# vliu15/speech-masters-thesis

Measured on AMD Instinct MI355X. Metric: LJSpeech utterances/sec per VQ-VAE train step, higher is better.
Workload: dtype bf16

## Files before the change

### include/smt_hip.h

```cpp
#ifndef SMT_HIP_H
#define SMT_HIP_H

#include <stddef.h>
#include <stdint.h>

#ifdef __cplusplus
extern "C" {
#endif

typedef void* smt_stream_t;

enum { SMT_F32 = 0, SMT_BF16 = 1 };

const char* smt_last_error(void);
int smt_abi_version(void);

size_t smt_vq_prep_bytes(int k_bins, int dim);
int smt_vq_prepare(const float* codebook, int k_bins, int dim, void* prep, size_t prep_bytes, smt_stream_t stream);

size_t smt_vq_forward_workspace_bytes(int64_t n_rows, int k_bins, int dim);
int smt_vq_forward(const float* x, const float* codebook, void* prep, const float* row_mask,
                   int64_t n_rows, int k_bins, int dim,
                   int64_t* idx, float* min_dist, float* x_d, float* sums,
                   void* workspace, size_t workspace_bytes, smt_stream_t stream);
// ... 56 lines not shown
  const int* lens_in2;
  int c_in2, ld_x2;
  int64_t bs_x2;
  const uint32_t* drop_keys_dev;
  int drop_keys_dev_stride;
} smt_conv_desc;
int smt_conv1d_ntc(const smt_conv_desc* desc, smt_stream_t stream);
const char* smt_conv1d_kernel_name(const smt_conv_desc* desc);

size_t smt_conv1d_wgrad_workspace_bytes(const smt_conv_desc* desc);
int smt_conv1d_wgrad(const smt_conv_desc* desc, float* dweight, int64_t stride_out, int64_t stride_in,
                     int64_t stride_tap, const int* tap_map, float* dbias, void* workspace,
                     size_t workspace_bytes, smt_stream_t stream);
int smt_wgrad_reduce_defer(int on, smt_stream_t stream);
const char* smt_conv1d_wgrad_kernel_name(const smt_conv_desc* desc);

size_t smt_conv1x1_bwd_workspace_bytes(const smt_conv_desc* desc);
int smt_conv1x1_bwd(const smt_conv_desc* desc, float* dweight, int64_t stride_out, int64_t stride_in, float* dbias,
                    void* workspace, size_t workspace_bytes, smt_stream_t stream);

size_t smt_conv_k1_bwd_workspace_bytes(int batch, int t);
int smt_conv_k1_bwd(const void* dh, int64_t bs_dh, int ld_dh, const void* x, int64_t bs_x, int ld_x,
                    const void* w_packed_bwd, const void* res, int64_t bs_res, int ld_res, void* dx, int64_t bs_dx,
                    int ld_dx, const int* lens, int batch, int t, const void* zero_page, float* dweight,
                    int64_t stride_out, int64_t stride_in, float* dbias, void* workspace, size_t workspace_bytes,
                    smt_stream_t stream);

int smt_convt4s2(const void* x, int64_t bs_x, int ld_x, const void* w_packed, const float* bias, void* y, int64_t bs_y,
                 int ld_y, const int* lens_in, const int* lens_out, int batch, int t_in, int c_out, const void* zero_page,
                 smt_stream_t stream);
int smt_conv4s2(const void* x, int64_t bs_x, int ld_x, const void* w_packed, const float* bias, void* y, int64_t bs_y,
                int ld_y, const int* lens_in, const int* lens_out, int batch, int t_in, int c_in, const void* zero_page,
                smt_stream_t stream);

// ... 137 lines not shown
```

### speech-masters-thesis_amd/csrc/common.hip

```cpp
#include <stdarg.h>

#include "smt_common.h"

namespace smt {
static thread_local char g_err[512] = "";
void set_error(const char* fmt, ...) {
  va_list ap;
  va_start(ap, fmt);
  vsnprintf(g_err, sizeof(g_err), fmt, ap);
  va_end(ap);
}
}

extern "C" const char* smt_last_error(void) { return smt::g_err; }
extern "C" int smt_abi_version(void) { return 5; }
```

### speech-masters-thesis_amd/csrc/conv1x1_bwd.hip

```cpp
#include <algorithm>

#include "conv_common.h"

namespace smt {

struct Bwd1x1Args {
  const void* dy; const void* u; const void* w; void* dx; float* slab;
  const int* lens_out;
  long long dy_bs, u_bs, dx_bs;
  int lddy, ldu, lddx;
  int B, T, tiles_per_batch, tiles_per_wg, with_bias;
  float scale;
};

constexpr int FB_ROWS = 128, FB_C = 128, FB_ROWB = FB_C * 2, FB_TILE = FB_ROWS * FB_ROWB, FB_NT = 512;
constexpr int FB_NDX = 2 * 2;

__device__ __forceinline__ int fb_swz(int row) { return ((row & 3) << 2) | ((row >> 2) & 3); }

__device__ __forceinline__ bf16x8 fb_tr2(const unsigned char* pa, const unsigned char* pb) {
  s16x4 lo = __builtin_amdgcn_ds_read_tr16_b64_v4i16((__attribute__((address_space(3))) s16x4*)pa);
  s16x4 hi = __builtin_amdgcn_ds_read_tr16_b64_v4i16((__attribute__((address_space(3))) s16x4*)pb);
  typedef short s16x8 __attribute__((ext_vector_type(8)));
  s16x8 v = {lo[0], lo[1], lo[2], lo[3], hi[0], hi[1], hi[2], hi[3]};
  return __builtin_bit_cast(bf16x8, v);
}

__global__ __launch_bounds__(FB_NT) void conv1x1_bwd_kernel(Bwd1x1Args p) {
  typedef __bf16 T;
  extern __shared__ __attribute__((aligned(1024))) unsigned char smem[];
  const int tid = threadIdx.x, lane = tid & 63, wave = tid >> 6;
  const int wm = wave >> 2, wn = wave & 3;
  const int r = lane & 31, hh = lane >> 5;

  const int ntiles = p.tiles_per_batch * p.B;
  const int nwg = gridDim.x;
  const int wg = (blockIdx.x & 7) * (nwg >> 3) + (blockIdx.x >> 3);
  const int tile_begin = min(ntiles, wg * p.tiles_per_wg);
  const int tile_end = min(ntiles, tile_begin + p.tiles_per_wg);

  bf16x8 wfrag[FB_C / 16];
  {
    const int ci = wn * 32 + r;
    const unsigned char* wrow = reinterpret_cast<const unsigned char*>(p.w) + (size_t)ci * FB_ROWB;
#pragma unroll
    for (int kk = 0; kk < FB_C / 16; ++kk)
      wfrag[kk] = *reinterpret_cast<const bf16x8*>(wrow + (((2 * kk + hh) ^ (ci & 15)) << 4));
  }

  float bsum[2] = {0.f, 0.f};
  f32x16 accw[2];
#pragma unroll
// ... 131 lines not shown
      out[(size_t)row * FB_C + wn * 32 + r] = accw[j][e];
    }
#pragma unroll
  for (int j = 0; j < 2; ++j) {
    const float other = __shfl_xor(bsum[j], 32);
    if (hh == 0) out[(size_t)(64 + 32 * j + r) * FB_C + 32 * wn] = bsum[j] + other;
  }
}

static int bwd1x1_nwg(const smt_conv_desc* d) {
  const long long ntiles = (long long)((d->t_out + FB_ROWS - 1) / FB_ROWS) * d->batch;
  long long nwg = std::min<long long>(256, std::max<long long>(8, (ntiles + fused_min_tpw() - 1) / fused_min_tpw()));
  return (int)((nwg + 7) / 8 * 8);
}

}

using namespace smt;

static bool bwd1x1_ok(const smt_conv_desc* d) {
  return d->dtype == SMT_BF16 && d->taps == 1 && d->c_in == FB_C && d->c_out == FB_C && d->stride == 1 &&
         d->dilation == 1 && d->padding == 0 && d->out_stride == 1 && d->out_offset == 0 && d->t_in == d->t_out &&
         d->t_y == d->t_out && d->w_swizzled && d->zero_page && d->act_grad && d->act_grad_src && !d->res &&
         !d->act_out && !d->bias && !d->lens_in;
}

extern "C" size_t smt_conv1x1_bwd_workspace_bytes(const smt_conv_desc* d) {
  if (!d) return 0;
  return (size_t)bwd1x1_nwg(d) * 2 * 2 * 64 * FB_C * sizeof(float);
}

extern "C" int smt_conv1x1_bwd(const smt_conv_desc* d, float* dweight, int64_t stride_out, int64_t stride_in,
                               float* dbias, void* workspace, size_t workspace_bytes, smt_stream_t stream_) {
  hipStream_t stream = (hipStream_t)stream_;
  SMT_CHECK_ARG(d && d->x && d->y && d->w && dweight && workspace, "smt_conv1x1_bwd: null pointer");
  SMT_CHECK_ARG(bwd1x1_ok(d),
                "smt_conv1x1_bwd: needs the bf16 1x1 data-gradient descriptor of a 128->128 layer (swizzled weights, "
                "zero_page, act_grad set, no bias/res/act_out/lens_in)");
  SMT_CHECK_ARG(d->ld_x % 8 == 0 && d->ld_y % 8 == 0 && d->ld_act % 8 == 0, "smt_conv1x1_bwd: row pitches must keep 16-byte alignment");
  SMT_CHECK_ARG(workspace_bytes >= smt_conv1x1_bwd_workspace_bytes(d), "smt_conv1x1_bwd: workspace too small");
  const int nwg = bwd1x1_nwg(d);
  if (d->batch > 0 && d->t_out > 0) {
    Bwd1x1Args a;
    a.dy = d->x; a.u = d->act_grad_src; a.w = d->w; a.dx = d->y; a.slab = (float*)workspace;
    a.lens_out = d->lens_out;
    a.dy_bs = d->bs_x; a.u_bs = d->bs_act; a.dx_bs = d->bs_y;
    a.lddy = d->ld_x; a.ldu = d->ld_act; a.lddx = d->ld_y;
    a.B = d->batch; a.T = d->t_out;
    a.tiles_per_batch = (d->t_out + FB_ROWS - 1) / FB_ROWS;
    const long long ntiles = (long long)a.tiles_per_batch * d->batch;
    a.tiles_per_wg = (int)((ntiles + nwg - 1) / nwg);
    a.with_bias = dbias ? 1 : 0;
    a.scale = d->drop_scale;
    (void)hipFuncSetAttribute((const void*)conv1x1_bwd_kernel, hipFuncAttributeMaxDynamicSharedMemorySize, 160 * 1024);
    conv1x1_bwd_kernel<<<nwg, FB_NT, 4 * FB_TILE, stream>>>(a);
    SMT_CHECK_LAUNCH("conv1x1_bwd");
  }
  const int jmap[1] = {0};
  const int n_chunks = (d->batch > 0 && d->t_out > 0) ? nwg : 0;
  return launch_wgrad_reduce((const float*)workspace, dweight, dbias, n_chunks, 2, 1, 1, FB_C, FB_C, FB_C, stride_out,
                             stride_in, 0, jmap, stream, 4);
}
```

### speech-masters-thesis_amd/csrc/conv_wgrad.hip

```cpp
#include <algorithm>
#include <cstdlib>

#include "conv_common.h"

namespace smt {

struct WgradArgs {
  const void* x; const void* dy; float* slab;
  const int* lens_in;
  long long x_bs, dy_bs;
  int ldx, ldy;
  int B, Tin, Tout, Ty, Cin, Cout;
  int taps, stride, dil, pad, out_stride, out_offset;
  int rows_per_chunk, chunks_per_batch, nblk_ci, nblk_co, with_bias;
  int rs;
  int win, xstride;
};

template <typename T> struct WTr;
template <> struct WTr<__bf16> {
  static constexpr int R = 128;
  static constexpr int pitch(int ch) { return ch + 32; }
};
template <> struct WTr<float> {
// ... 309 lines not shown
    }
  }
}

struct ShiftArgs {
  const void* x; const void* dy; float* slab; const int* lens_in;
  long long x_bs, dy_bs;
  int ldx, ldy;
  int B, Tin, Tout, pad, rs;
  int tiles_per_item, tiles_per_wg, n_chunks, nblk_ci, nblk_co, with_bias;
};

constexpr int SH_R = 128, SH_XROWS = SH_R + 8, SH_DY = SH_R * 128, SH_X = SH_XROWS * 256, SH_STAGE = SH_DY + SH_X;

template <int NTAPS>
__global__ __launch_bounds__(512) void conv_wgrad_shift_kernel(ShiftArgs p, const __bf16* __restrict__ zero_page) {
  typedef __bf16 T;
  constexpr int CB = 64, CIB = 128, WNC = 4, NTHR = 512, DYB = CB * 2, XB = CIB * 2, PLANES = NTAPS + 1;
  extern __shared__ __attribute__((aligned(16))) unsigned char smem[];
  const int tid = threadIdx.x, lane = tid & 63, wave = tid >> 6;
  const int wm = wave / WNC, wn = wave % WNC;
  const int r = lane & 31, hh = lane >> 5;

  const int nblk = p.nblk_ci * p.nblk_co;
  const int xcd = blockIdx.x & 7, q = blockIdx.x >> 3;
  const int blk = q % nblk;
  const int cgl = (q / nblk) * 8 + xcd;
  if (cgl >= p.n_chunks) return;
  const int co0 = (blk / p.nblk_ci) * CB, ci0 = (blk % p.nblk_ci) * CIB;
  const int ntiles = p.tiles_per_item * p.B * p.rs;
  const int tile_begin = cgl * p.tiles_per_wg;
  const int tile_end = min(ntiles, tile_begin + p.tiles_per_wg);
  const int rs = p.rs;
  const bool bias_plane = p.with_bias && (ci0 == 0);

  f32x16 acc[PLANES];
#pragma unroll
  for (int j = 0; j < PLANES; ++j)
#pragma unroll
    for (int e = 0; e < 16; ++e) acc[j][e] = 0.f;

  auto stage = [&](int tile, int buf) {
// ... 80 lines not shown
          bw = u32x4{w[m], w[m + 1], w[m + 2], w[m + 3]};
        }
        acc[s] = __builtin_amdgcn_mfma_f32_32x32x16_bf16(a, __builtin_bit_cast(bf16x8, bw), acc[s], 0, 0, 0);
      }
      if (bias_plane && (k0 & 3) == wn) acc[NTAPS] = __builtin_amdgcn_mfma_f32_32x32x16_bf16(a, ones, acc[NTAPS], 0, 0, 0);
    }
  }
  float* out = p.slab + ((size_t)cgl * nblk + blk) * (size_t)PLANES * CB * CIB;
#pragma unroll
  for (int j = 0; j < PLANES; ++j)
#pragma unroll
    for (int e = 0; e < 16; ++e) {
      const int row = wm * 32 + (e & 3) + 8 * (e >> 2) + 4 * hh;
      out[((size_t)j * CB + row) * CIB + wn * 32 + r] = acc[j][e];
    }
}

struct ShiftPlan { int rs, pad, tiles_per_item, tiles_per_wg, n_chunks, nblk_co, nblk_ci; };
static bool wgrad_shift_plan(const smt_conv_desc* d, ShiftPlan* pl) {
  static const bool off = getenv("SMT_WGRAD_NO_SHIFT") != nullptr;
  if (off || d->dtype != SMT_BF16 || d->stride != 1 || d->out_stride != 1 || d->out_offset != 0 || !d->zero_page ||
      d->c_in % 128 != 0 || d->c_out % 64 != 0 || d->taps < 3 || d->taps > 9 || !(d->taps & 1) || d->t_in != d->t_out)
    return false;
  int rs = 1, pad = d->padding;
  if (d->dilation > 1) {
    static const int min_rows = getenv("SMT_CLASS_MIN_ROWS") ? atoi(getenv("SMT_CLASS_MIN_ROWS")) : 128;
    if (d->padding % d->dilation != 0 || d->t_out / d->dilation < min_rows) return false;
    rs = d->dilation; pad = d->padding / d->dilation;
  }
  if (pad < 0 || pad > d->taps - 1) return false;
// ... 381 lines not shown
  SMT_CHECK_ARG(workspace_bytes >= smt_conv1d_wgrad_workspace_bytes(d), "smt_conv1d_wgrad: workspace too small");
  smt_conv_desc wv;
  if (wgrad_window_desc(d, &wv))
    return wgrad_window(d, &wv, dweight, stride_out, stride_in, stride_tap, tap_map, dbias, workspace, workspace_bytes, stream);
  size_t off = 0;
  for (int j0 = 0; j0 < d->taps; j0 += WG_GROUP) {
    smt_conv_desc g = wgrad_group_desc(d, j0, std::min(WG_GROUP, d->taps - j0));
    const size_t need = align_up(wgrad_group_ws(&g), 256);
    int rc = wgrad_group(&g, dweight, stride_out, stride_in, stride_tap, tap_map + j0, j0 == 0 ? dbias : nullptr,
                         (char*)workspace + off, need, stream);
    if (rc) return rc;
    off += need;
  }
  return 0;
}
```

### speech-masters-thesis_amd/smt_amd/convops.py

```python
import contextlib
import ctypes
import functools
import weakref
from dataclasses import dataclass
from typing import Optional

import torch

from . import native as N
from . import profiler

SMT_F32, SMT_BF16 = 0, 1
_DT = {torch.float32: SMT_F32, torch.bfloat16: SMT_BF16}


class ConvDesc(ctypes.Structure):
    _fields_ = [("dtype", ctypes.c_int), ("batch", ctypes.c_int), ("t_in", ctypes.c_int), ("t_out", ctypes.c_int),
                ("t_y", ctypes.c_int), ("c_in", ctypes.c_int), ("c_out", ctypes.c_int), ("taps", ctypes.c_int),
                ("stride", ctypes.c_int), ("dilation", ctypes.c_int), ("padding", ctypes.c_int),
                ("out_stride", ctypes.c_int), ("out_offset", ctypes.c_int), ("act_out", ctypes.c_int),
                ("act_grad", ctypes.c_int), ("site_width", ctypes.c_int), ("ld_x", ctypes.c_int),
                ("ld_y", ctypes.c_int), ("ld_res", ctypes.c_int), ("ld_act", ctypes.c_int), ("ld_yact", ctypes.c_int),
                ("drop_keys", ctypes.c_uint32 * 8), ("drop_thresh16", ctypes.c_uint32), ("drop_scale", ctypes.c_float),
                ("bs_x", ctypes.c_int64), ("bs_y", ctypes.c_int64), ("bs_res", ctypes.c_int64),
# ... 271 lines not shown


@contextlib.contextmanager
def reduce_batch(device):
    lib = N.lib()
    with N.workspace.arena(device):
        N.check(lib.smt_wgrad_reduce_defer(1, N.stream_ptr()), "smt_wgrad_reduce_defer")
        try:
            yield
        finally:
            with profiler.region("conv_wgrad_reduce", bound="hbm"):
                N.check(lib.smt_wgrad_reduce_defer(0, N.stream_ptr()), "smt_wgrad_reduce_defer")


_K3GATE = not bool(int(__import__("os").environ.get("SMT_NO_K3GATE", "0")))


def _conv_k3gate(u2, x, w3p, w1p, b3, b1, z, g, lens32):
    b, t = x.shape[0], x.shape[1]
    (pu, bsu, ldu), (px, bsx, ldx_), (pz, bsz, ldz), (pg, bsg, ldg) = _geom(u2), _geom(x), _geom(z), _geom(g)
    rows = float(b) * t
    with profiler.region("conv_k3gate", flops=2.0 * rows * 512 * (128 + 64), nbytes=rows * (1024 + 128) * 2, bound="hbm",
                         dtype="bf16"):
        N.check(N.lib().smt_conv_k3gate_fwd(pu, bsu, ldu, px, bsx, ldx_, _p(w3p), _p(w1p), _p(b3), _p(b1), pz, bsz, ldz, pg,
                                            bsg, ldg, _p(lens32), b, t, _p(_zero_page(x.device)), N.stream_ptr()),
                "smt_conv_k3gate_fwd")


def _pack_cat_bwd(weights, dtype):
    n_in = weights[0].shape[1]
# ... 88 lines not shown
    name = lib.smt_conv1d_wgrad_kernel_name(ctypes.byref(desc)).decode() + ("_" + _tag(desc) if profiler.DETAIL else "")
    with profiler.region(name, flops=_conv_flops(desc), bound="mfma", dtype=dtype):
        N.check(lib.smt_conv1d_wgrad(ctypes.byref(desc), _p(dweight), s_out, s_in, s_tap, arr, _p(dbias), _p(ws),
                                     ws.numel(), N.stream_ptr()), "smt_conv1d_wgrad")


def _conv1x1_bwd(desc, dweight, s_out, s_in, dbias):
    lib = N.lib()
    ws_bytes = lib.smt_conv1x1_bwd_workspace_bytes(ctypes.byref(desc))
    ws = N.workspace.get(ws_bytes, dweight.device)
    rows = float(desc.batch) * desc.t_out
    name = "conv1x1_bwd" + ("_" + _tag(desc) if profiler.DETAIL else "")
    with profiler.region(name, flops=2 * _conv_flops(desc), nbytes=rows * 3 * desc.c_in * 2, bound="hbm", dtype="bf16"):
        N.check(lib.smt_conv1x1_bwd(ctypes.byref(desc), _p(dweight), s_out, s_in, _p(dbias), _p(ws), ws.numel(),
                                    N.stream_ptr()), "smt_conv1x1_bwd")


def _conv_gate_bwd(dy, g, w_packed_bwd, dx, lens32, dweight, dbias):
    lib = N.lib()
    b, t = g.shape[0], g.shape[1]
    ws = N.workspace.get(lib.smt_conv_gate_bwd_workspace_bytes(b, t), g.device)
    (pdy, bsdy, lddy), (pg, bsg, ldg), (pdx, bsdx, lddx) = _geom(dy), _geom(g), _geom(dx)
    rows = float(b) * t
    with profiler.region("conv_gate_bwd", flops=4.0 * rows * 64 * 64, nbytes=rows * 3 * 64 * 2, bound="hbm", dtype="bf16"):
        N.check(lib.smt_conv_gate_bwd(pdy, bsdy, lddy, pg, bsg, ldg, _p(w_packed_bwd), pdx, bsdx, lddx, _p(lens32), b, t,
                                      _p(_zero_page(g.device)), _p(dweight), dweight.stride(0), dweight.stride(1),
                                      _p(dbias), _p(ws), ws.numel(), N.stream_ptr()), "smt_conv_gate_bwd")


def _conv_k1_bwd(dh, x, w_packed_bwd, res, dx, lens32, dweight, dbias):
# ... 403 lines not shown
        grads[6 * depth], grads[6 * depth + 1] = torch.empty_like(wg), f32(bg.shape)
        if dt == torch.bfloat16 and w == 64:
            _conv_gate_bwd(dout, g, _pack_bwd(wg, dt), dg, lens32, grads[6 * depth], grads[6 * depth + 1])
        else:
            d = _dgrad_stride1(dout, _pack_bwd(wg, dt), dg, 1, 1, 0)
            d.lens_out = _p(lens32)
            _launch(d, "conv_dgrad", _conv_flops(d), _conv_bytes(d, x.element_size()))
            _wgrad(_base_desc(g, dout, lens32, w, w, 1, 1, 1, 0, t), grads[6 * depth], w, 1, 1, [0], grads[6 * depth + 1])

        dz = torch.empty_like(z)
        with profiler.region("gate_mix_bwd", nbytes=z.numel() * z.element_size() * 2.125, bound="hbm"):
            N.check(N.lib().smt_gate_mix_bwd(_p(z), _p(dg), _p(dz), _DT[dt], b * t, w, depth, depth * c2, w, depth * c2,
                                             N.stream_ptr()), "smt_gate_mix_bwd")
        del dg
        dh1 = torch.empty_like(z)
        dh2 = torch.empty(b, t, c2, dtype=dt, device=dev)
        for dd, (k, dil, pad) in enumerate(geometry):
            sl = slice(dd * c2, (dd + 1) * c2)
            w1, b1, w2, b2, w3, b3 = br[dd]
            dz_d, u1_d, u2_d = dz[:, :, sl], u1[:, :, sl], u2[:, :, sl]
            dma = _dma_ok(dt, c2, c2)
            wb3 = _pack_bwd(w3, dt, dma)
            d = _dgrad_stride1(dz_d, wb3, dh2, 1, 1, 0)
            if dma:
                _use_dma(d, wb3)
            _set_act_grad(d, u2_d, scale)
            grads[6 * dd + 4], grads[6 * dd + 5] = torch.empty_like(w3), f32(b3.shape)
            if dma and c2 == 128:
                _conv1x1_bwd(d, grads[6 * dd + 4], c2, 1, grads[6 * dd + 5])
            else:
                _launch(d, "conv_dgrad", _conv_flops(d), _conv_bytes(d, x.element_size()))
                _wgrad(_base_desc(u2_d, dz_d, None, c2, c2, 1, 1, 1, 0, t), grads[6 * dd + 4], c2, 1, 1, [0],
                       grads[6 * dd + 5])
            wb2 = _pack_bwd(w2, dt, dma)
            d = _dgrad_stride1(dh2, wb2, dh1[:, :, sl], k, dil, pad)
            if dma:
                _use_dma(d, wb2)
            _set_act_grad(d, u1_d, scale)
            d.res, d.bs_res, d.ld_res = _geom(dz_d)
            _launch(d, "conv_dgrad", _conv_flops(d), _conv_bytes(d, x.element_size()))
            grads[6 * dd + 2], grads[6 * dd + 3] = torch.empty_like(w2), f32(b2.shape)
            _wgrad(_base_desc(u1_d, dh2, None, c2, c2, k, 1, dil, pad, t), grads[6 * dd + 2], c2 * k, k, 1,
                   list(range(k)), grads[6 * dd + 3])
        del dz, dh2
        dx = torch.empty_like(x)
        dw1cat, db1cat = torch.empty(depth * c2, w, 1, dtype=torch.float32, device=dev), f32((depth * c2,))
        if dt == torch.bfloat16 and w == 64 and depth * c2 == 512:
            _conv_k1_bwd(dh1, x, _pack_cat_bwd([p[0] for p in br], dt), dout, dx, lens32, dw1cat, db1cat)
        else:
            d = _dgrad_stride1(dh1, _pack_cat_bwd([p[0] for p in br], dt), dx, 1, 1, 0)
            d.lens_out = _p(lens32)
            d.res, d.bs_res, d.ld_res = _geom(dout)
            _launch(d, "conv_dgrad", _conv_flops(d), _conv_bytes(d, x.element_size()))
            _wgrad(_base_desc(x, dh1, lens32, w, depth * c2, 1, 1, 1, 0, t), dw1cat, w, 1, 1, [0], db1cat)
        for dd in range(depth):
            grads[6 * dd] = dw1cat[dd * c2:(dd + 1) * c2]
            grads[6 * dd + 1] = db1cat[dd * c2:(dd + 1) * c2]
        return (dx, None, None, None, None, *grads)


def gated_hifi_block(x, lens, geometry, params, *, p_drop, training, seed, site_base):
    return _GatedHiFi.apply(x, lens, tuple(geometry), (p_drop, training, seed, site_base), len(params), *params)
```

### speech-masters-thesis_amd/smt_amd/native.py

```python
import contextlib
import ctypes
import os
import threading

import torch

_HERE = os.path.dirname(os.path.abspath(__file__))
LIB_PATH = os.environ.get("SMT_HIP_LIB") or os.path.join(_HERE, "libsmt_hip.so")
ABI_VERSION = 5

_lib = None
_lock = threading.Lock()

c_i64 = ctypes.c_int64
c_int = ctypes.c_int
c_f32 = ctypes.c_float
c_u32 = ctypes.c_uint32
c_ptr = ctypes.c_void_p
c_size = ctypes.c_size_t

_SIGNATURES = {
    "smt_last_error": (ctypes.c_char_p, []),
    "smt_abi_version": (c_int, []),
    "smt_vq_forward_workspace_bytes": (c_size, [c_i64, c_int, c_int]),
# ... 1 lines not shown
    "smt_vq_prepare": (c_int, [c_ptr, c_int, c_int, c_ptr, c_size, c_ptr]),
    "smt_vq_forward": (c_int, [c_ptr, c_ptr, c_ptr, c_ptr, c_i64, c_int, c_int, c_ptr, c_ptr, c_ptr, c_ptr, c_ptr, c_size,
                               c_ptr]),
    "smt_vq_backward": (c_int, [c_ptr, c_ptr, c_ptr, c_ptr, c_ptr, c_ptr, c_i64, c_int, c_ptr, c_ptr]),
    "smt_vq_ema_accumulate_workspace_bytes": (c_size, [c_i64, c_int, c_int]),
    "smt_vq_ema_accumulate": (c_int, [c_ptr, c_ptr, c_ptr, c_i64, c_int, c_int, c_ptr, c_ptr, c_size, c_ptr]),
    "smt_vq_ema_apply": (c_int, [c_ptr, c_ptr, c_ptr, c_ptr, c_ptr, c_f32, c_f32, c_int, c_int, c_ptr, c_ptr, c_size,
                                 c_ptr]),
    "smt_pack_weight": (c_int, [c_ptr, c_ptr, c_int, c_int, c_int, c_int, c_i64, c_i64, c_i64, c_ptr, c_int, c_ptr]),
    "smt_pack_weights_batched": (c_int, [c_ptr, c_ptr, c_ptr, c_int, c_ptr]),
    "smt_conv1d_ntc": (c_int, [c_ptr, c_ptr]),
    "smt_conv1d_kernel_name": (ctypes.c_char_p, [c_ptr]),
    "smt_conv1d_wgrad_workspace_bytes": (c_size, [c_ptr]),
    "smt_conv1d_wgrad_kernel_name": (ctypes.c_char_p, [c_ptr]),
    "smt_conv1d_wgrad": (c_int, [c_ptr, c_ptr, c_i64, c_i64, c_i64, c_ptr, c_ptr, c_ptr, c_size, c_ptr]),
    "smt_wgrad_reduce_defer": (c_int, [c_int, c_ptr]),
    "smt_conv1x1_bwd_workspace_bytes": (c_size, [c_ptr]),
    "smt_conv1x1_bwd": (c_int, [c_ptr, c_ptr, c_i64, c_i64, c_ptr, c_ptr, c_size, c_ptr]),
    "smt_conv_gate_bwd_workspace_bytes": (c_size, [c_int, c_int]),
    "smt_conv_gate_bwd": (c_int, [c_ptr, c_i64, c_int, c_ptr, c_i64, c_int, c_ptr, c_ptr, c_i64, c_int, c_ptr, c_int,
                                  c_int, c_ptr, c_ptr, c_i64, c_i64, c_ptr, c_ptr, c_size, c_ptr]),
    "smt_conv_k1_bwd_workspace_bytes": (c_size, [c_int, c_int]),
    "smt_conv_k1_bwd": (c_int, [c_ptr, c_i64, c_int, c_ptr, c_i64, c_int, c_ptr, c_ptr, c_i64, c_int, c_ptr, c_i64,
                                c_int, c_ptr, c_int, c_int, c_ptr, c_ptr, c_i64, c_i64, c_ptr, c_ptr, c_size, c_ptr]),
    "smt_convt4s2": (c_int, [c_ptr, c_i64, c_int, c_ptr, c_ptr, c_ptr, c_i64, c_int, c_ptr, c_ptr, c_int, c_int, c_int, c_ptr, c_ptr]),
    "smt_conv4s2": (c_int, [c_ptr, c_i64, c_int, c_ptr, c_ptr, c_ptr, c_i64, c_int, c_ptr, c_ptr, c_int, c_int, c_int, c_ptr, c_ptr]),
    "smt_conv_k3gate_fwd": (c_int, [c_ptr, c_i64, c_int, c_ptr, c_i64, c_int, c_ptr, c_ptr, c_ptr, c_ptr, c_ptr, c_i64, c_int,
                                    c_ptr, c_i64, c_int, c_ptr, c_int, c_int, c_ptr, c_ptr]),
    "smt_gate_mix_fwd": (c_int, [c_ptr, c_ptr, c_int, c_i64, c_int, c_int, c_int, c_int, c_ptr]),
    "smt_gate_mix_bwd": (c_int, [c_ptr, c_ptr, c_ptr, c_int, c_i64, c_int, c_int, c_int, c_int, c_int, c_ptr]),
    "smt_conv_in_fwd": (c_int, [c_ptr, c_ptr, c_ptr, c_ptr, c_ptr, c_int, c_int, c_int, c_int, c_int, c_int, c_int,
                                c_int, c_ptr]),
    "smt_conv_in_wgrad_workspace_bytes": (c_size, [c_int, c_int, c_int]),
# ... 152 lines not shown
```

Measured before the change: 493.6.

## Batch gated-block branch backward kernels into single multi-branch launches

Adds multi-branch variants of the fused 1x1 data/weight-gradient kernel and the shifted weight-gradient kernel. Each one launch covers all four dilation branches, with workgroups split across branches in proportion to their work. Python's gated HiFi backward uses these when the bf16, c2=128, depth=4 conditions hold. The goal is to cut per-branch launch overhead and fill the GPU better on small per-branch grids. The cost is fewer workgroups per branch and a per-block runtime switch on tap count.

```diff
diff --git a/include/smt_hip.h b/include/smt_hip.h
--- a/include/smt_hip.h
+++ b/include/smt_hip.h
@@ -94,10 +94,18 @@
                      size_t workspace_bytes, smt_stream_t stream);
 int smt_wgrad_reduce_defer(int on, smt_stream_t stream);
 const char* smt_conv1d_wgrad_kernel_name(const smt_conv_desc* desc);
+const char* smt_conv1d_wgrad_branches_kernel_name(const smt_conv_desc* desc, int n_branches);
+size_t smt_conv1d_wgrad_branches_workspace_bytes(const smt_conv_desc* desc, int n_branches);
+int smt_conv1d_wgrad_branches(const smt_conv_desc* desc, int n_branches, float* const* dweight, float* const* dbias,
+                              void* workspace, size_t workspace_bytes, smt_stream_t stream);
 
 size_t smt_conv1x1_bwd_workspace_bytes(const smt_conv_desc* desc);
 int smt_conv1x1_bwd(const smt_conv_desc* desc, float* dweight, int64_t stride_out, int64_t stride_in, float* dbias,
                     void* workspace, size_t workspace_bytes, smt_stream_t stream);
+size_t smt_conv1x1_bwd_branches_workspace_bytes(const smt_conv_desc* desc, int n_branches);
+int smt_conv1x1_bwd_branches(const smt_conv_desc* desc, int n_branches, const void* const* w_branches, float* const* dweight,
+                             float* const* dbias, int64_t stride_out, int64_t stride_in, void* workspace,
+                             size_t workspace_bytes, smt_stream_t stream);
 
 size_t smt_conv_k1_bwd_workspace_bytes(int batch, int t);
 int smt_conv_k1_bwd(const void* dh, int64_t bs_dh, int ld_dh, const void* x, int64_t bs_x, int ld_x,
diff --git a/speech-masters-thesis_amd/csrc/common.hip b/speech-masters-thesis_amd/csrc/common.hip
--- a/speech-masters-thesis_amd/csrc/common.hip
+++ b/speech-masters-thesis_amd/csrc/common.hip
@@ -13,4 +13,4 @@
 }
 
 extern "C" const char* smt_last_error(void) { return smt::g_err; }
-extern "C" int smt_abi_version(void) { return 5; }
+extern "C" int smt_abi_version(void) { return 6; }
diff --git a/speech-masters-thesis_amd/csrc/conv1x1_bwd.hip b/speech-masters-thesis_amd/csrc/conv1x1_bwd.hip
--- a/speech-masters-thesis_amd/csrc/conv1x1_bwd.hip
+++ b/speech-masters-thesis_amd/csrc/conv1x1_bwd.hip
@@ -1,8 +1,11 @@
 #include <algorithm>
+#include <numeric>
 
 #include "conv_common.h"
 
 namespace smt {
+
+constexpr int FB_MAXBR = 4;
 
 struct Bwd1x1Args {
   const void* dy; const void* u; const void* w; void* dx; float* slab;
@@ -11,6 +14,9 @@
   int lddy, ldu, lddx;
   int B, T, tiles_per_batch, tiles_per_wg, with_bias;
   float scale;
+  const void* wbr[FB_MAXBR];
+  long long slab_br;
+  int nwg_br;
 };
 
 constexpr int FB_ROWS = 128, FB_C = 128, FB_ROWB = FB_C * 2, FB_TILE = FB_ROWS * FB_ROWB, FB_NT = 512;
@@ -26,6 +32,7 @@
   return __builtin_bit_cast(bf16x8, v);
 }
 
+template <bool BRANCHES>
 __global__ __launch_bounds__(FB_NT) void conv1x1_bwd_kernel(Bwd1x1Args p) {
   typedef __bf16 T;
   extern __shared__ __attribute__((aligned(1024))) unsigned char smem[];
@@ -35,7 +42,16 @@
 
   const int ntiles = p.tiles_per_batch * p.B;
   const int nwg = gridDim.x;
-  const int wg = (blockIdx.x & 7) * (nwg >> 3) + (blockIdx.x >> 3);
+  int wg = (blockIdx.x & 7) * (nwg >> 3) + (blockIdx.x >> 3);
+  if constexpr (BRANCHES) {
+    const int br = wg / p.nwg_br;
+    wg -= br * p.nwg_br;
+    p.dy = reinterpret_cast<const T*>(p.dy) + br * FB_C;
+    p.u = reinterpret_cast<const T*>(p.u) + br * FB_C;
+    p.dx = reinterpret_cast<T*>(p.dx) + br * FB_C;
+    p.w = br == 0 ? p.wbr[0] : br == 1 ? p.wbr[1] : br == 2 ? p.wbr[2] : p.wbr[3];
+    p.slab += br * p.slab_br;
+  }
   const int tile_begin = min(ntiles, wg * p.tiles_per_wg);
   const int tile_end = min(ntiles, tile_begin + p.tiles_per_wg);
 
@@ -197,6 +213,13 @@
   return (int)((nwg + 7) / 8 * 8);
 }
 
+static int bwd1x1_nwg_br(const smt_conv_desc* d, int nbr) {
+  const long long ntiles = (long long)((d->t_out + FB_ROWS - 1) / FB_ROWS) * d->batch;
+  const int cap = 256 / nbr, unit = 8 / std::gcd(8, nbr);
+  long long n = std::min<long long>(cap, std::max<long long>(1, (ntiles + fused_min_tpw() - 1) / fused_min_tpw()));
+  return (int)((n + unit - 1) / unit * unit);
+}
+
 }
 
 using namespace smt;
@@ -208,9 +231,27 @@
          !d->act_out && !d->bias && !d->lens_in;
 }
 
+static size_t bwd1x1_slab_bytes(int nwg) { return (size_t)nwg * 2 * 2 * 64 * FB_C * sizeof(float); }
+
+static void bwd1x1_args(const smt_conv_desc* d, Bwd1x1Args& a, void* workspace, int nwg, bool with_bias) {
+  a.dy = d->x; a.u = d->act_grad_src; a.w = d->w; a.dx = d->y; a.slab = (float*)workspace;
+  a.lens_out = d->lens_out;
+  a.dy_bs = d->bs_x; a.u_bs = d->bs_act; a.dx_bs = d->bs_y;
+  a.lddy = d->ld_x; a.ldu = d->ld_act; a.lddx = d->ld_y;
+  a.B = d->batch; a.T = d->t_out;
+  a.tiles_per_batch = (d->t_out + FB_ROWS - 1) / FB_ROWS;
+  const long long ntiles = (long long)a.tiles_per_batch * d->batch;
+  a.tiles_per_wg = (int)((ntiles + nwg - 1) / nwg);
+  a.with_bias = with_bias ? 1 : 0;
+  a.scale = d->drop_scale;
+  for (int j = 0; j < FB_MAXBR; ++j) a.wbr[j] = d->w;
+  a.slab_br = 0;
+  a.nwg_br = nwg;
+}
+
 extern "C" size_t smt_conv1x1_bwd_workspace_bytes(const smt_conv_desc* d) {
   if (!d) return 0;
-  return (size_t)bwd1x1_nwg(d) * 2 * 2 * 64 * FB_C * sizeof(float);
+  return bwd1x1_slab_bytes(bwd1x1_nwg(d));
 }
 
 extern "C" int smt_conv1x1_bwd(const smt_conv_desc* d, float* dweight, int64_t stride_out, int64_t stride_in,
@@ -225,18 +266,9 @@
   const int nwg = bwd1x1_nwg(d);
   if (d->batch > 0 && d->t_out > 0) {
     Bwd1x1Args a;
-    a.dy = d->x; a.u = d->act_grad_src; a.w = d->w; a.dx = d->y; a.slab = (float*)workspace;
-    a.lens_out = d->lens_out;
-    a.dy_bs = d->bs_x; a.u_bs = d->bs_act; a.dx_bs = d->bs_y;
-    a.lddy = d->ld_x; a.ldu = d->ld_act; a.lddx = d->ld_y;
-    a.B = d->batch; a.T = d->t_out;
-    a.tiles_per_batch = (d->t_out + FB_ROWS - 1) / FB_ROWS;
-    const long long ntiles = (long long)a.tiles_per_batch * d->batch;
-    a.tiles_per_wg = (int)((ntiles + nwg - 1) / nwg);
-    a.with_bias = dbias ? 1 : 0;
-    a.scale = d->drop_scale;
-    (void)hipFuncSetAttribute((const void*)conv1x1_bwd_kernel, hipFuncAttributeMaxDynamicSharedMemorySize, 160 * 1024);
-    conv1x1_bwd_kernel<<<nwg, FB_NT, 4 * FB_TILE, stream>>>(a);
+    bwd1x1_args(d, a, workspace, nwg, dbias != nullptr);
+    (void)hipFuncSetAttribute((const void*)conv1x1_bwd_kernel<false>, hipFuncAttributeMaxDynamicSharedMemorySize, 160 * 1024);
+    conv1x1_bwd_kernel<false><<<nwg, FB_NT, 4 * FB_TILE, stream>>>(a);
     SMT_CHECK_LAUNCH("conv1x1_bwd");
   }
   const int jmap[1] = {0};
@@ -244,3 +276,49 @@
   return launch_wgrad_reduce((const float*)workspace, dweight, dbias, n_chunks, 2, 1, 1, FB_C, FB_C, FB_C, stride_out,
                              stride_in, 0, jmap, stream, 4);
 }
+
+extern "C" size_t smt_conv1x1_bwd_branches_workspace_bytes(const smt_conv_desc* d, int n_branches) {
+  if (!d || n_branches < 1 || n_branches > FB_MAXBR) return 0;
+  return (size_t)n_branches * align_up(bwd1x1_slab_bytes(bwd1x1_nwg_br(d, n_branches)), 256);
+}
+
+extern "C" int smt_conv1x1_bwd_branches(const smt_conv_desc* d, int n_branches, const void* const* w_branches,
+                                        float* const* dweight, float* const* dbias, int64_t stride_out, int64_t stride_in,
+                                        void* workspace, size_t workspace_bytes, smt_stream_t stream_) {
+  hipStream_t stream = (hipStream_t)stream_;
+  SMT_CHECK_ARG(n_branches >= 1 && n_branches <= FB_MAXBR, "smt_conv1x1_bwd_branches: 1..%d branches", FB_MAXBR);
+  SMT_CHECK_ARG(d && d->x && d->y && w_branches && dweight && dbias && workspace, "smt_conv1x1_bwd_branches: null pointer");
+  for (int j = 0; j < n_branches; ++j)
+    SMT_CHECK_ARG(w_branches[j] && dweight[j], "smt_conv1x1_bwd_branches: null pointer (branch %d)", j);
+  SMT_CHECK_ARG(bwd1x1_ok(d),
+                "smt_conv1x1_bwd_branches: needs the bf16 1x1 data-gradient descriptor of branch 0's 128->128 layer (swizzled "
+                "weights, zero_page, act_grad set, no bias/res/act_out/lens_in)");
+  SMT_CHECK_ARG(d->ld_x % 8 == 0 && d->ld_y % 8 == 0 && d->ld_act % 8 == 0,
+                "smt_conv1x1_bwd_branches: row pitches must keep 16-byte alignment");
+  SMT_CHECK_ARG(d->ld_x >= n_branches * FB_C && d->ld_y >= n_branches * FB_C && d->ld_act >= n_branches * FB_C,
+                "smt_conv1x1_bwd_branches: branch j's channels are %d j further along every row: rows too short", FB_C);
+  SMT_CHECK_ARG(workspace_bytes >= smt_conv1x1_bwd_branches_workspace_bytes(d, n_branches),
+                "smt_conv1x1_bwd_branches: workspace too small");
+  const int nwg_br = bwd1x1_nwg_br(d, n_branches);
+  const size_t slab_br = align_up(bwd1x1_slab_bytes(nwg_br), 256);
+  const bool live = d->batch > 0 && d->t_out > 0;
+  if (live) {
+    Bwd1x1Args a;
+    bwd1x1_args(d, a, workspace, nwg_br, dbias[0] != nullptr);
+    for (int j = 0; j < FB_MAXBR; ++j) a.wbr[j] = w_branches[std::min(j, n_branches - 1)];
+    a.slab_br = (long long)(slab_br / sizeof(float));
+    for (int j = 1; j < n_branches; ++j)
+      SMT_CHECK_ARG((dbias[j] != nullptr) == (dbias[0] != nullptr), "smt_conv1x1_bwd_branches: give every branch a bias or none");
+    (void)hipFuncSetAttribute((const void*)conv1x1_bwd_kernel<true>, hipFuncAttributeMaxDynamicSharedMemorySize, 160 * 1024);
+    conv1x1_bwd_kernel<true><<<nwg_br * n_branches, FB_NT, 4 * FB_TILE, stream>>>(a);
+    SMT_CHECK_LAUNCH("conv1x1_bwd");
+  }
+  const int jmap[1] = {0};
+  for (int j = 0; j < n_branches; ++j) {
+    const int rc = launch_wgrad_reduce((const float*)((char*)workspace + j * slab_br), dweight[j], dbias[j],
+                                       live ? nwg_br : 0, 2, 1, 1, FB_C, FB_C, FB_C, stride_out, stride_in, 0, jmap, stream,
+                                       4);
+    if (rc) return rc;
+  }
+  return 0;
+}
diff --git a/speech-masters-thesis_amd/csrc/conv_wgrad.hip b/speech-masters-thesis_amd/csrc/conv_wgrad.hip
--- a/speech-masters-thesis_amd/csrc/conv_wgrad.hip
+++ b/speech-masters-thesis_amd/csrc/conv_wgrad.hip
@@ -347,7 +347,7 @@
 constexpr int SH_R = 128, SH_XROWS = SH_R + 8, SH_DY = SH_R * 128, SH_X = SH_XROWS * 256, SH_STAGE = SH_DY + SH_X;
 
 template <int NTAPS>
-__global__ __launch_bounds__(512) void conv_wgrad_shift_kernel(ShiftArgs p, const __bf16* __restrict__ zero_page) {
+__device__ __forceinline__ void wgrad_shift_body(const ShiftArgs& p, const __bf16* __restrict__ zero_page, int cgl, int blk) {
   typedef __bf16 T;
   constexpr int CB = 64, CIB = 128, WNC = 4, NTHR = 512, DYB = CB * 2, XB = CIB * 2, PLANES = NTAPS + 1;
   extern __shared__ __attribute__((aligned(16))) unsigned char smem[];
@@ -356,9 +356,6 @@
   const int r = lane & 31, hh = lane >> 5;
 
   const int nblk = p.nblk_ci * p.nblk_co;
-  const int xcd = blockIdx.x & 7, q = blockIdx.x >> 3;
-  const int blk = q % nblk;
-  const int cgl = (q / nblk) * 8 + xcd;
   if (cgl >= p.n_chunks) return;
   const int co0 = (blk / p.nblk_ci) * CB, ci0 = (blk % p.nblk_ci) * CIB;
   const int ntiles = p.tiles_per_item * p.B * p.rs;
@@ -469,6 +466,37 @@
       const int row = wm * 32 + (e & 3) + 8 * (e >> 2) + 4 * hh;
       out[((size_t)j * CB + row) * CIB + wn * 32 + r] = acc[j][e];
     }
+}
+
+template <int NTAPS>
+__global__ __launch_bounds__(512) void conv_wgrad_shift_kernel(ShiftArgs p, const __bf16* __restrict__ zero_page) {
+  const int nblk = p.nblk_ci * p.nblk_co;
+  const int xcd = blockIdx.x & 7, q = blockIdx.x >> 3;
+  wgrad_shift_body<NTAPS>(p, zero_page, (q / nblk) * 8 + xcd, q % nblk);
+}
+
+constexpr int SHB_MAXBR = 4;
+struct ShiftBranches {
+  int n, nblk;
+  int taps[SHB_MAXBR], slot0[SHB_MAXBR];
+  ShiftArgs br[SHB_MAXBR];
+};
+
+__global__ __launch_bounds__(512) void conv_wgrad_shift_branches_kernel(ShiftBranches bt, const __bf16* __restrict__ zero_page) {
+  const int xcd = blockIdx.x & 7, q = blockIdx.x >> 3;
+  const int blk = q % bt.nblk, slot = (q / bt.nblk) * 8 + xcd;
+  int j = 0;
+#pragma unroll
+  for (int k = 1; k < SHB_MAXBR; ++k)
+    if (k < bt.n && slot >= bt.slot0[k]) j = k;
+  const ShiftArgs& a = bt.br[j];
+  const int cgl = slot - bt.slot0[j];
+  switch (bt.taps[j]) {
+    case 3: wgrad_shift_body<3>(a, zero_page, cgl, blk); break;
+    case 5: wgrad_shift_body<5>(a, zero_page, cgl, blk); break;
+    case 7: wgrad_shift_body<7>(a, zero_page, cgl, blk); break;
+    default: wgrad_shift_body<9>(a, zero_page, cgl, blk); break;
+  }
 }
 
 struct ShiftPlan { int rs, pad, tiles_per_item, tiles_per_wg, n_chunks, nblk_co, nblk_ci; };
@@ -880,3 +908,107 @@
   }
   return 0;
 }
+
+struct BranchPlan { int nblk, total_slots; int slots[SHB_MAXBR]; ShiftPlan pl[SHB_MAXBR]; size_t slab_bytes[SHB_MAXBR]; };
+
+static bool wgrad_branches_plan(const smt_conv_desc* d, int n, BranchPlan* bp) {
+  if (!d || n < 1 || n > SHB_MAXBR) return false;
+  long long ntiles[SHB_MAXBR], work[SHB_MAXBR], sum = 0;
+  for (int j = 0; j < n; ++j) {
+    ShiftPlan& pl = bp->pl[j];
+    if (!wgrad_shift_plan(&d[j], &pl) || pl.nblk_co != bp->pl[0].nblk_co || pl.nblk_ci != bp->pl[0].nblk_ci) return false;
+    ntiles[j] = (long long)pl.tiles_per_item * d[j].batch * pl.rs;
+    work[j] = ntiles[j] * d[j].taps;
+    sum += work[j];
+  }
+  bp->nblk = bp->pl[0].nblk_co * bp->pl[0].nblk_ci;
+  bp->total_slots = 256 / bp->nblk;
+  if (bp->total_slots < n || sum <= 0) return false;
+  int given = 0;
+  for (int j = 0; j < n; ++j) {
+    bp->slots[j] = std::max(1, (int)(bp->total_slots * work[j] / sum));
+    given += bp->slots[j];
+  }
+  while (given < bp->total_slots) {
+    int best = 0;
+    for (int j = 1; j < n; ++j)
+      if (work[j] * bp->slots[best] > work[best] * bp->slots[j]) best = j;
+    ++bp->slots[best]; ++given;
+  }
+  while (given > bp->total_slots) {
+    int best = -1;
+    for (int j = 0; j < n; ++j)
+      if (bp->slots[j] > 1 && (best < 0 || work[j] * bp->slots[best] < work[best] * bp->slots[j])) best = j;
+    --bp->slots[best]; --given;
+  }
+  for (int j = 0; j < n; ++j) {
+    ShiftPlan& pl = bp->pl[j];
+    pl.tiles_per_wg = (int)((ntiles[j] + bp->slots[j] - 1) / bp->slots[j]);
+    pl.n_chunks = (int)((ntiles[j] + pl.tiles_per_wg - 1) / pl.tiles_per_wg);
+    bp->slab_bytes[j] = align_up((size_t)pl.n_chunks * bp->nblk * (d[j].taps + 1) * 64 * 128 * sizeof(float), 256);
+  }
+  return true;
+}
+
+extern "C" const char* smt_conv1d_wgrad_branches_kernel_name(const smt_conv_desc* d, int n_branches) {
+  BranchPlan bp;
+  return wgrad_branches_plan(d, n_branches, &bp) ? "conv_wgrad_shift" : "";
+}
+
+extern "C" size_t smt_conv1d_wgrad_branches_workspace_bytes(const smt_conv_desc* d, int n_branches) {
+  BranchPlan bp;
+  if (!wgrad_branches_plan(d, n_branches, &bp)) return 0;
+  size_t total = 0;
+  for (int j = 0; j < n_branches; ++j) total += bp.slab_bytes[j];
+  return total;
+}
+
+extern "C" int smt_conv1d_wgrad_branches(const smt_conv_desc* d, int n_branches, float* const* dweight, float* const* dbias,
+                                         void* workspace, size_t workspace_bytes, smt_stream_t stream_) {
+  hipStream_t stream = (hipStream_t)stream_;
+  SMT_CHECK_ARG(d && dweight && dbias && workspace, "smt_conv1d_wgrad_branches: null pointer");
+  BranchPlan bp;
+  SMT_CHECK_ARG(wgrad_branches_plan(d, n_branches, &bp),
+                "smt_conv1d_wgrad_branches: every branch must be a shifted-fragment weight gradient with the same channel "
+                "blocks (smt_conv1d_wgrad_branches_kernel_name returns \"\" otherwise: run smt_conv1d_wgrad per branch)");
+  SMT_CHECK_ARG(workspace_bytes >= smt_conv1d_wgrad_branches_workspace_bytes(d, n_branches),
+                "smt_conv1d_wgrad_branches: workspace too small");
+  ShiftBranches bt;
+  bt.n = n_branches; bt.nblk = bp.nblk;
+  size_t off = 0;
+  int slot0 = 0;
+  const void* zero_page = d[0].zero_page;
+  for (int j = 0; j < SHB_MAXBR; ++j) {
+    const int jj = std::min(j, n_branches - 1);
+    const smt_conv_desc& dj = d[jj];
+    const ShiftPlan& pl = bp.pl[jj];
+    if (j < n_branches) {
+      SMT_CHECK_ARG(dj.x && dj.y && dweight[j], "smt_conv1d_wgrad_branches: null pointer (branch %d)", j);
+      SMT_CHECK_ARG(dj.ld_x % 8 == 0 && dj.ld_y % 8 == 0, "smt_conv1d_wgrad_branches: pitches must keep 16-byte alignment");
+    }
+    ShiftArgs& a = bt.br[j];
+    a.x = dj.x; a.dy = dj.y; a.slab = (float*)((char*)workspace + off); a.lens_in = dj.lens_in;
+    a.x_bs = dj.bs_x; a.dy_bs = dj.bs_y; a.ldx = dj.ld_x; a.ldy = dj.ld_y;
+    a.B = dj.batch; a.Tin = dj.t_in; a.Tout = dj.t_out; a.pad = pl.pad; a.rs = pl.rs;
+    a.tiles_per_item = pl.tiles_per_item; a.tiles_per_wg = pl.tiles_per_wg; a.n_chunks = pl.n_chunks;
+    a.nblk_ci = pl.nblk_ci; a.nblk_co = pl.nblk_co; a.with_bias = dbias[jj] ? 1 : 0;
+    bt.taps[j] = dj.taps;
+    bt.slot0[j] = slot0;
+    if (j < n_branches) { off += bp.slab_bytes[j]; slot0 += bp.slots[j]; }
+  }
+  dim3 grid((unsigned)(8 * ((bp.total_slots + 7) / 8) * bp.nblk));
+  (void)hipFuncSetAttribute((const void*)conv_wgrad_shift_branches_kernel, hipFuncAttributeMaxDynamicSharedMemorySize,
+                            160 * 1024);
+  conv_wgrad_shift_branches_kernel<<<grid, 512, 2 * SH_STAGE, stream>>>(bt, (const __bf16*)zero_page);
+  SMT_CHECK_LAUNCH("conv_wgrad_shift");
+  for (int j = 0; j < n_branches; ++j) {
+    const smt_conv_desc& dj = d[j];
+    int jmap[16];
+    for (int t = 0; t < 16; ++t) jmap[t] = t;
+    const int rc = launch_wgrad_reduce(bt.br[j].slab, dweight[j], dbias[j], bp.pl[j].n_chunks, bp.pl[j].nblk_co,
+                                       bp.pl[j].nblk_ci, dj.taps, dj.c_in, dj.c_out, 128, (long long)dj.c_in * dj.taps, dj.taps,
+                                       1, jmap, stream, 4);
+    if (rc) return rc;
+  }
+  return 0;
+}
diff --git a/speech-masters-thesis_amd/smt_amd/convops.py b/speech-masters-thesis_amd/smt_amd/convops.py
--- a/speech-masters-thesis_amd/smt_amd/convops.py
+++ b/speech-masters-thesis_amd/smt_amd/convops.py
@@ -309,6 +309,7 @@
 
 
 _K3GATE = not bool(int(__import__("os").environ.get("SMT_NO_K3GATE", "0")))
+_BRANCH_WGRAD = not bool(int(__import__("os").environ.get("SMT_NO_BRANCH_WGRAD", "0")))
 
 
 def _conv_k3gate(u2, x, w3p, w1p, b3, b1, z, g, lens32):
@@ -427,6 +428,40 @@
     with profiler.region(name, flops=2 * _conv_flops(desc), nbytes=rows * 3 * desc.c_in * 2, bound="hbm", dtype="bf16"):
         N.check(lib.smt_conv1x1_bwd(ctypes.byref(desc), _p(dweight), s_out, s_in, _p(dbias), _p(ws), ws.numel(),
                                     N.stream_ptr()), "smt_conv1x1_bwd")
+
+
+def _conv1x1_bwd_branches(desc, w_packed, dweights, dbiases, s_out, s_in):
+    lib = N.lib()
+    n = len(w_packed)
+    ws = N.workspace.get(lib.smt_conv1x1_bwd_branches_workspace_bytes(ctypes.byref(desc), n), dweights[0].device)
+    wp = (ctypes.c_void_p * n)(*[t.data_ptr() for t in w_packed])
+    dw = (ctypes.c_void_p * n)(*[t.data_ptr() for t in dweights])
+    db = (ctypes.c_void_p * n)(*[t.data_ptr() for t in dbiases])
+    rows = float(desc.batch) * desc.t_out
+    name = "conv1x1_bwd" + ("_" + _tag(desc) if profiler.DETAIL else "")
+    with profiler.region(name, flops=2 * n * _conv_flops(desc), nbytes=n * rows * 3 * desc.c_in * 2, bound="hbm", dtype="bf16"):
+        N.check(lib.smt_conv1x1_bwd_branches(ctypes.byref(desc), n, wp, dw, db, s_out, s_in, _p(ws), ws.numel(),
+                                             N.stream_ptr()), "smt_conv1x1_bwd_branches")
+
+
+def _wgrad_branches(descs, dweights, dbiases):
+    lib = N.lib()
+    n = len(descs)
+    for d in descs:
+        d.zero_page = _p(_zero_page(dweights[0].device))
+    arr = (ConvDesc * n)(*descs)
+    name = lib.smt_conv1d_wgrad_branches_kernel_name(arr, n).decode()
+    if not name:
+        for d, dw, db in zip(descs, dweights, dbiases):
+            _wgrad(d, dw, d.c_in * d.taps, d.taps, 1, list(range(d.taps)), db)
+        return
+    ws = N.workspace.get(lib.smt_conv1d_wgrad_branches_workspace_bytes(arr, n), dweights[0].device)
+    dw = (ctypes.c_void_p * n)(*[t.data_ptr() for t in dweights])
+    db = (ctypes.c_void_p * n)(*[t.data_ptr() for t in dbiases])
+    name = name + ("_" + "+".join(_tag(d) for d in descs) if profiler.DETAIL else "")
+    with profiler.region(name, flops=sum(_conv_flops(d) for d in descs), bound="mfma", dtype="bf16"):
+        N.check(lib.smt_conv1d_wgrad_branches(arr, n, dw, db, _p(ws), ws.numel(), N.stream_ptr()),
+                "smt_conv1d_wgrad_branches")
 
 
 def _conv_gate_bwd(dy, g, w_packed_bwd, dx, lens32, dweight, dbias):
@@ -860,35 +895,39 @@
                                              N.stream_ptr()), "smt_gate_mix_bwd")
         del dg
         dh1 = torch.empty_like(z)
-        dh2 = torch.empty(b, t, c2, dtype=dt, device=dev)
-        for dd, (k, dil, pad) in enumerate(geometry):
-            sl = slice(dd * c2, (dd + 1) * c2)
-            w1, b1, w2, b2, w3, b3 = br[dd]
-            dz_d, u1_d, u2_d = dz[:, :, sl], u1[:, :, sl], u2[:, :, sl]
-            dma = _dma_ok(dt, c2, c2)
-            wb3 = _pack_bwd(w3, dt, dma)
-            d = _dgrad_stride1(dz_d, wb3, dh2, 1, 1, 0)
-            if dma:
-                _use_dma(d, wb3)
-            _set_act_grad(d, u2_d, scale)
-            grads[6 * dd + 4], grads[6 * dd + 5] = torch.empty_like(w3), f32(b3.shape)
-            if dma and c2 == 128:
-                _conv1x1_bwd(d, grads[6 * dd + 4], c2, 1, grads[6 * dd + 5])
-            else:
+        if _BRANCH_WGRAD and dt == torch.bfloat16 and c2 == 128 and depth == 4:
+            _GatedHiFi._branches_backward(dz, u1, u2, dh1, br, grads, geometry, scale)
+        else:
+            dh2 = torch.empty(b, t, c2, dtype=dt, device=dev)
+            for dd, (k, dil, pad) in enumerate(geometry):
+                sl = slice(dd * c2, (dd + 1) * c2)
+                w1, b1, w2, b2, w3, b3 = br[dd]
+                dz_d, u1_d, u2_d = dz[:, :, sl], u1[:, :, sl], u2[:, :, sl]
+                dma = _dma_ok(dt, c2, c2)
+                wb3 = _pack_bwd(w3, dt, dma)
+                d = _dgrad_stride1(dz_d, wb3, dh2, 1, 1, 0)
+                if dma:
+                    _use_dma(d, wb3)
+                _set_act_grad(d, u2_d, scale)
+                grads[6 * dd + 4], grads[6 * dd + 5] = torch.empty_like(w3), f32(b3.shape)
+                if dma and c2 == 128:
+                    _conv1x1_bwd(d, grads[6 * dd + 4], c2, 1, grads[6 * dd + 5])
+                else:
+                    _launch(d, "conv_dgrad", _conv_flops(d), _conv_bytes(d, x.element_size()))
+                    _wgrad(_base_desc(u2_d, dz_d, None, c2, c2, 1, 1, 1, 0, t), grads[6 * dd + 4], c2, 1, 1, [0],
+                           grads[6 * dd + 5])
+                wb2 = _pack_bwd(w2, dt, dma)
+                d = _dgrad_stride1(dh2, wb2, dh1[:, :, sl], k, dil, pad)
+                if dma:
+                    _use_dma(d, wb2)
+                _set_act_grad(d, u1_d, scale)
+                d.res, d.bs_res, d.ld_res = _geom(dz_d)
                 _launch(d, "conv_dgrad", _conv_flops(d), _conv_bytes(d, x.element_size()))
-                _wgrad(_base_desc(u2_d, dz_d, None, c2, c2, 1, 1, 1, 0, t), grads[6 * dd + 4], c2, 1, 1, [0],
-                       grads[6 * dd + 5])
-            wb2 = _pack_bwd(w2, dt, dma)
-            d = _dgrad_stride1(dh2, wb2, dh1[:, :, sl], k, dil, pad)
-            if dma:
-                _use_dma(d, wb2)
-            _set_act_grad(d, u1_d, scale)
-            d.res, d.bs_res, d.ld_res = _geom(dz_d)
-            _launch(d, "conv_dgrad", _conv_flops(d), _conv_bytes(d, x.element_size()))
-            grads[6 * dd + 2], grads[6 * dd + 3] = torch.empty_like(w2), f32(b2.shape)
-            _wgrad(_base_desc(u1_d, dh2, None, c2, c2, k, 1, dil, pad, t), grads[6 * dd + 2], c2 * k, k, 1,
-                   list(range(k)), grads[6 * dd + 3])
-        del dz, dh2
+                grads[6 * dd + 2], grads[6 * dd + 3] = torch.empty_like(w2), f32(b2.shape)
+                _wgrad(_base_desc(u1_d, dh2, None, c2, c2, k, 1, dil, pad, t), grads[6 * dd + 2], c2 * k, k, 1,
+                       list(range(k)), grads[6 * dd + 3])
+            del dh2
+        del dz
         dx = torch.empty_like(x)
         dw1cat, db1cat = torch.empty(depth * c2, w, 1, dtype=torch.float32, device=dev), f32((depth * c2,))
         if dt == torch.bfloat16 and w == 64 and depth * c2 == 512:
@@ -904,6 +943,35 @@
             grads[6 * dd + 1] = db1cat[dd * c2:(dd + 1) * c2]
         return (dx, None, None, None, None, *grads)
 
+    @staticmethod
+    def _branches_backward(dz, u1, u2, dh1, br, grads, geometry, scale):
+        t = dz.shape[1]
+        c2 = dz.shape[2] // len(geometry)
+        dt, dev = dz.dtype, dz.device
+        dh2 = torch.empty_like(dz)
+        wb3 = [_pack_bwd(p[4], dt, True) for p in br]
+        d = _dgrad_stride1(dz[:, :, :c2], wb3[0], dh2[:, :, :c2], 1, 1, 0)
+        _use_dma(d, wb3[0])
+        _set_act_grad(d, u2[:, :, :c2], scale)
+        for dd, p in enumerate(br):
+            grads[6 * dd + 4] = torch.empty_like(p[4])
+            grads[6 * dd + 5] = torch.empty(p[5].shape, dtype=torch.float32, device=dev)
+        _conv1x1_bwd_branches(d, wb3, [grads[6 * dd + 4] for dd in range(len(br))],
+                              [grads[6 * dd + 5] for dd in range(len(br))], c2, 1)
+        wdescs = []
+        for dd, (k, dil, pad) in enumerate(geometry):
+            sl = slice(dd * c2, (dd + 1) * c2)
+            wb2 = _pack_bwd(br[dd][2], dt, True)
+            d = _dgrad_stride1(dh2[:, :, sl], wb2, dh1[:, :, sl], k, dil, pad)
+            _use_dma(d, wb2)
+            _set_act_grad(d, u1[:, :, sl], scale)
+            d.res, d.bs_res, d.ld_res = _geom(dz[:, :, sl])
+            _launch(d, "conv_dgrad", _conv_flops(d), _conv_bytes(d, dz.element_size()))
+            grads[6 * dd + 2] = torch.empty_like(br[dd][2])
+            grads[6 * dd + 3] = torch.empty(br[dd][3].shape, dtype=torch.float32, device=dev)
+            wdescs.append(_base_desc(u1[:, :, sl], dh2[:, :, sl], None, c2, c2, k, 1, dil, pad, t))
+        _wgrad_branches(wdescs, [grads[6 * dd + 2] for dd in range(len(br))], [grads[6 * dd + 3] for dd in range(len(br))])
+
 
 def gated_hifi_block(x, lens, geometry, params, *, p_drop, training, seed, site_base):
     return _GatedHiFi.apply(x, lens, tuple(geometry), (p_drop, training, seed, site_base), len(params), *params)
diff --git a/speech-masters-thesis_amd/smt_amd/native.py b/speech-masters-thesis_amd/smt_amd/native.py
--- a/speech-masters-thesis_amd/smt_amd/native.py
+++ b/speech-masters-thesis_amd/smt_amd/native.py
@@ -7,7 +7,7 @@
 
 _HERE = os.path.dirname(os.path.abspath(__file__))
 LIB_PATH = os.environ.get("SMT_HIP_LIB") or os.path.join(_HERE, "libsmt_hip.so")
-ABI_VERSION = 5
+ABI_VERSION = 6
 
 _lib = None
 _lock = threading.Lock()
@@ -39,9 +39,14 @@
     "smt_conv1d_wgrad_workspace_bytes": (c_size, [c_ptr]),
     "smt_conv1d_wgrad_kernel_name": (ctypes.c_char_p, [c_ptr]),
     "smt_conv1d_wgrad": (c_int, [c_ptr, c_ptr, c_i64, c_i64, c_i64, c_ptr, c_ptr, c_ptr, c_size, c_ptr]),
+    "smt_conv1d_wgrad_branches_kernel_name": (ctypes.c_char_p, [c_ptr, c_int]),
+    "smt_conv1d_wgrad_branches_workspace_bytes": (c_size, [c_ptr, c_int]),
+    "smt_conv1d_wgrad_branches": (c_int, [c_ptr, c_int, c_ptr, c_ptr, c_ptr, c_size, c_ptr]),
     "smt_wgrad_reduce_defer": (c_int, [c_int, c_ptr]),
     "smt_conv1x1_bwd_workspace_bytes": (c_size, [c_ptr]),
     "smt_conv1x1_bwd": (c_int, [c_ptr, c_ptr, c_i64, c_i64, c_ptr, c_ptr, c_size, c_ptr]),
+    "smt_conv1x1_bwd_branches_workspace_bytes": (c_size, [c_ptr, c_int]),
+    "smt_conv1x1_bwd_branches": (c_int, [c_ptr, c_int, c_ptr, c_ptr, c_ptr, c_i64, c_i64, c_ptr, c_size, c_ptr]),
     "smt_conv_gate_bwd_workspace_bytes": (c_size, [c_int, c_int]),
     "smt_conv_gate_bwd": (c_int, [c_ptr, c_i64, c_int, c_ptr, c_i64, c_int, c_ptr, c_ptr, c_i64, c_int, c_ptr, c_int,
                                   c_int, c_ptr, c_ptr, c_i64, c_i64, c_ptr, c_ptr, c_size, c_ptr]),
```

Result: slower. 478.8 (median of 2 runs) (-3.0%).
